# zju3dv/RelightableAvatar

Hardware: AMD Instinct MI355X
Metric: rays_per_sec (higher is better)
Workload: dtype f16

## Files before the change

### relightableavatar_amd/csrc/ra_api.cpp

```cpp
#include "ra_api_impl.hpp"
#include <cmath>

int check_ready(ra_ctx* c, const char* who) {
    if (!c) { ra_set_error(std::string(who) + ": null ctx"); return 1; }
    if (!c->have_weights) { ra_set_error(std::string(who) + ": weights not finalized"); return 1; }
    if (!c->have_frame) { ra_set_error(std::string(who) + ": no frame set (ra_set_frame)"); return 1; }
    if (hipSetDevice(c->device) != hipSuccess) { ra_set_error(std::string(who) + ": hipSetDevice failed"); return 1; }
    return 0;
}

static void zero_chunk_counters(ra_ctx* c, hipStream_t s) {
    hipMemsetAsync(icnt(c, 0), 0, CNT_ALL * sizeof(int), s);
    c->fc_next = 0;
    c->fc_wrapped = false;
    c->cnt_zero = true;
}
int* next_fine_counter(ra_ctx* c, hipStream_t s) {
    if (c->fc_next >= CNT_FC_SLOTS) {
        hipMemsetAsync(icnt(c, CNT_FC0), 0, CNT_FC_SLOTS * sizeof(int), s);
        c->fc_next = 0;
        c->fc_wrapped = true;
    }
    return icnt(c, CNT_FC0 + c->fc_next++);
}
// ... 90 lines not shown
static int key_mask_from(ra_ctx* c, const float* probe, int ph, int pw, hipStream_t s) {
    if (c->key_external) return 0;
    c->key_valid = false;
    if (!key_tier(c) || !probe) return 0;
    if (c->key_mask.ensure((size_t)c->n_lights) || c->key_share.ensure((size_t)c->n_lights * sizeof(float))) return 1;
    launch_key_lights(probe, 1, ph, pw, c->light_dir.as<float>(), c->light_area.as<float>(), c->n_lights, c->cfg.key_light_share, KEY_LIGHTS_MAX, 0,
                      c->key_share.as<float>(), c->key_mask.as<unsigned char>(), s);
    c->key_valid = true;
    return 0;
}

static void fine_level(ra_ctx* c, const MlpIO& io, int n, bool comp, hipStream_t s, int hint = -1) {
    const int nv = variant_size(n, hint);
    if (comp) {
        Timer t(c, s, T_K3C);
        launch_mlp_sdf_comp(c->host.geo, c->sarena_c.p, c->barena.as<float>(), c->fr, io, nv, s, c->k3cc_ok, grid_size(n, nv));
    } else {
        Timer t(c, s, k3_waves(nv) == 8 ? T_K3_WIDE : T_K3_NARROW);
        k3_launch(c, io, nv, s, grid_size(n, nv));
    }
}

static int hdq_pass(ra_ctx* c, const RaySet& rs, int n, float th, int smooth, float* sdf, hipStream_t s, int what = Q_OTHER,
                    const unsigned char* key = nullptr, int n_key = 0) {
    if (n <= 0) return 0;
    int err = 0;
    int* fine_idx = c->buf<int>("fine_idx", n, &err);
    float* bpts = c->buf<float>("fine_bpts", (size_t)n * 3, &err);
    if (err) return 1;
    HdqOut out{};
    out.sdf = sdf; out.fine_count = next_fine_counter(c, s); out.fine_idx = fine_idx; out.bpts = bpts;
    const int hint = fine_hint(c, c->fc_next - 1);
    int hint2 = -1;
    if (key && n_key > 0) {
        out.key = key;
        out.fine_idx2 = c->buf<int>("fine_idx_k", n_key, &err);
        out.bpts2 = c->buf<float>("fine_bpts_k", (size_t)n_key * 3, &err);
        if (err) return 1;
        out.fine_count2 = next_fine_counter(c, s);
        hint2 = fine_hint(c, c->fc_next - 1);
    }
    out.counters = dcnt(c);
    launch_hdq_coarse(c->fr, rs, n, th, c->cfg.blend_radius, out, s, c->cfg.use_geodesic_filter != 0);
    MlpIO io{};
    io.bpts = bpts; io.idx = fine_idx; io.count = out.fine_count; io.sdf = sdf; io.dist_th = th; io.smooth = smooth;
    io.resd_limit = c->cfg.resd_limit; io.counters = dcnt(c);
    fine_level(c, io, n, precise(c, what), s, hint);
    if (out.key) {
        io.bpts = out.bpts2; io.idx = out.fine_idx2; io.count = out.fine_count2;
        fine_level(c, io, n_key, true, s, hint2);
    }
    return 0;
}

int full_query(ra_ctx* c, FullIO io, int n, hipStream_t s) {
    const bool gated = c->gate && n > 65536;
    if (gated && c->gate->armed) RA_HIP(hipStreamWaitEvent(s, c->gate->done, 0));
    struct Release {
        ra_ctx* c; hipStream_t s; bool on;
        ~Release() { if (on) { hipEventRecord(c->gate->done, s); c->gate->armed = true; } }
    } release{c, s, gated};
    Timer t(c, s, T_K4);
    const int batch = c->cfg.k4_batch_slots > 0 ? c->cfg.k4_batch_slots : (1 << 20);
    const int cap = n < batch ? n : batch;
    int err = 0;
    char* tape = c->buf<char>("k4_tape", mlp_full_rev_tape_bytes(cap), &err);
    if (err) {
        ra_set_error("full query: no device memory for the activation tape (" + std::to_string(mlp_full_rev_tape_bytes(cap) >> 20) +
                     " MB): lower cfg.k4_batch_slots / cfg.volume_chunk_rays");
        return 1;
// ... 9 lines not shown
}

static int forward_pass(ra_ctx* c, const float* x, const float* v, int n, const int* n_dev, float th, float* raw, hipStream_t s) {
    if (n <= 0) return 0;
    int err = 0;
    const int C = raw_channels(c);
    int* fine_idx = c->buf<int>("fine_idx", n, &err);
    float* bpts = c->buf<float>("fine_bpts", (size_t)n * 3, &err);
    float* mats = c->buf<float>("fine_mats", (size_t)n * 24, &err);
    float* sdf = c->buf<float>("fwd_sdf", n, &err);
    if (err) return 1;
    RaySet rs{};
    rs.mode = 0; rs.x = x; rs.n_dev = n_dev;
    HdqOut out{};
    out.sdf = sdf; out.fine_count = next_fine_counter(c, s); out.fine_idx = fine_idx; out.bpts = bpts; out.mats = mats;
    out.raw_zero = raw; out.raw_C = C;
    out.counters = dcnt(c);
    launch_hdq_coarse(c->fr, rs, n, th, c->cfg.blend_radius, out, s, c->cfg.use_geodesic_filter != 0);
    FullIO io = full_io(c);
    io.bpts = bpts; io.mats = mats; io.view = v; io.idx = fine_idx; io.count = out.fine_count; io.raw = raw;
    return full_query(c, io, n, s);
}

static TraceState alloc_trace(ra_ctx* c, const std::string& p, int n, bool soft, int* err) {
    TraceState ts{};
    ts.t = c->buf<float>(p + "t", n, err);
    ts.d0 = c->buf<float>(p + "d0", n, err);
    ts.occ = c->buf<float>(p + "occ", n, err);
    ts.ot = c->buf<float>(p + "ot", n, err);
    ts.stuck = c->buf<unsigned char>(p + "stuck", n, err);
    if (!soft) {
        ts.dt = c->buf<float>(p + "dt", n, err);
        ts.st = c->buf<float>(p + "st", n, err);
        ts.cd = c->buf<float>(p + "cd", n, err);
        ts.off = c->buf<float>(p + "off", n, err);
        ts.rlx = c->buf<float>(p + "rlx", n, err);
    }
    return ts;
}

int sdf_points_precise(ra_ctx* c, int mode, const float* pts, int n, float dist_th, float* sdf, hipStream_t s) {
    if (n <= 0) return 0;
    if (mode == 2) {
        RaySet rs{};
        rs.mode = 0; rs.x = pts;
        return hdq_pass(c, rs, n, dist_th, 0, sdf, s, Q_PRECISE);
    }
    int err = 0;
    int* idx = c->buf<int>("fine_idx", n, &err);
    if (err) return 1;
    int* cnt = next_fine_counter(c, s);
    launch_iota(idx, n, cnt, s);
// ... 131 lines not shown
    ShadowGen g{};
    g.surf = st.surf; g.norm = st.norm_slots; g.acc = st.acc; g.hit_idx = st.hit_idx; g.hit_count = st.hit_count; g.ldir = c->light_dir.as<float>();
    for (int k = 0; k < 6; ++k) g.bbox[k] = st.bbox[k];
    g.n_boxes = st.n_boxes > 1 ? st.n_boxes : 0;
    for (int j = 0; j < g.n_boxes; ++j) {
        for (int k = 0; k < 6; ++k) g.boxes[j][k] = st.boxes[6 * j + k];
        g.box_start[j] = st.box_start[j];
    }
    if (g.n_boxes) g.box_start[g.n_boxes] = st.box_start[g.n_boxes];
    g.perm = g.n_boxes ? st.perm : nullptr;
    g.near_offset = st.near_offset; g.L = L; g.no_visibility = st.no_visibility; g.local_visibility = st.local_visibility;
    g.split_wide_groups = st.split_wide_groups ? 1 : 0;
    g.lvis = st.lvis; g.ldot = st.ldot;
    g.ray_count = icnt(c, CNT_RAYS);
    const bool traced = !(st.no_visibility || st.local_visibility);
    TraceState sh{};
    float* ssdf = nullptr;
    if (traced) {
        g.ray_pix = c->buf<int>("lv_pix", NR, &err);
        g.ray_light = c->buf<int>("lv_light", NR, &err);
        g.ray_slot = c->buf<int>("lv_slot", NR, &err);
        g.near_ = c->buf<float>("lv_near", NR, &err);
        g.far_ = c->buf<float>("lv_far", NR, &err);
        sh = alloc_trace(c, "sh_", (int)NR, shadow.soft_shadow != 0, &err);
        ssdf = c->buf<float>("sh_sdf", NR, &err);
    }
    const bool keyed = traced && key_tier(c) && c->key_valid;
    const size_t NK = keyed ? (size_t)P * (size_t)(L < KEY_LIGHTS_MAX ? L : KEY_LIGHTS_MAX) : 0;
    if (err) return 1;
    if (c->gate && c->gate->armed) RA_HIP(hipStreamWaitEvent(s, c->gate->done, 0));
    launch_shadow_gen(g, P, s, c->cnt_zero);
    c->cnt_zero = false;
    if (traced) {
        sh.near_ = g.near_; sh.far_ = g.far_; sh.tan_i = c->light_sharp.as<float>(); sh.light = g.ray_light;
        launch_trace_init(sh, (int)NR, g.ray_count, shadow, s);
        RaySet r2{};
        r2.mode = 2; r2.o = st.surf; r2.t = sh.t; r2.pix = g.ray_pix; r2.light = g.ray_light; r2.ldir = c->light_dir.as<float>();
        r2.n_dev = g.ray_count;
        r2.skip = c->cfg.query_skip ? sh.stuck : nullptr;
        r2.nn_hint = c->buf<int>("lv_nn", NR * 3, &err);
        if (err) return 1;
        for (int it = 0; it < shadow.iters; ++it) {
            r2.hint_valid = it > 0;
            r2.hint_src = it == 0 ? st.pix_nn : nullptr;
            r2.hint_src_index = it == 0 ? g.ray_pix : nullptr;
            if (hdq_pass(c, r2, (int)NR, shadow.dist_th, 1, ssdf, s, Q_OTHER, keyed ? c->key_mask.as<unsigned char>() : nullptr, (int)NK)) return 1;
            launch_trace_update(sh, ssdf, (int)NR, g.ray_count, it, shadow, s);
        }
        launch_shadow_scatter(sh.occ, g.ray_slot, g.ray_count, (int)NR, st.lvis, s);
        launch_accumulate(g.ray_count, &dcnt(c)->n_shadow_rays, s);
    }
    if (c->gate) { RA_HIP(hipEventRecord(c->gate->done, s)); c->gate->armed = true; }
    return 0;
}

int ra_begin_render(ra_ctx* c) {
    RA_CHECK(c, "ra_begin_render: null ctx");
    c->call_no = 0;
    return 0;
}

int ra_set_key_probes(ra_ctx* c, const float* probes, int n, int ph, int pw, int accumulate, void* stream) {
    RA_CHECK(c && n >= 0 && (n == 0 || (probes && ph > 0 && pw > 0)), "ra_set_key_probes: bad arguments");
    if (n == 0) { c->key_external = false; c->key_valid = false; return 0; }
    RA_CHECK(c->have_weights && c->n_lights > 0, "ra_set_key_probes: needs the relight network's light set (ra_finalize_weights)");
    RA_HIP(hipSetDevice(c->device));
    const bool acc = accumulate && c->key_external && c->key_valid;
    c->key_external = true;
    if (!key_tier(c)) { c->key_valid = false; return 0; }
    if (c->key_mask.ensure((size_t)c->n_lights) || c->key_share.ensure((size_t)c->n_lights * sizeof(float))) return 1;
    launch_key_lights(probes, n, ph, pw, c->light_dir.as<float>(), c->light_area.as<float>(), c->n_lights, c->cfg.key_light_share, KEY_LIGHTS_MAX,
                      acc ? 1 : 0, c->key_share.as<float>(), c->key_mask.as<unsigned char>(), (hipStream_t)stream);
    c->key_valid = true;
    RA_HIP(hipGetLastError());
    return 0;
// ... 289 lines not shown
```

### relightableavatar_amd/csrc/ra_hdq.hip

```cpp
#include "ra_kernels.hpp"
#include <type_traits>
#include <cstdlib>

namespace {

constexpr int KNN_THREADS = 256;

#ifdef RA_COARSE_TS
__device__ long long ra_coarse_ts[64 * 64 * 16 * 8];
extern "C" int ra_coarse_read_timestamps(long long* out) { return (int)hipMemcpyFromSymbol(out, HIP_SYMBOL(ra_coarse_ts), sizeof(ra_coarse_ts)); }
#define RA_CSTAMP(k) do { if (tsp) { __builtin_amdgcn_sched_barrier(0); if ((threadIdx.x & 63) == 0) tsp[k] = __builtin_readcyclecounter(); __builtin_amdgcn_sched_barrier(0); } } while (0)
#else
#define RA_CSTAMP(k) do { } while (0)
#endif
constexpr int VT = 2048;

__device__ __forceinline__ void inv3d(const float R[9], float M[9]) {
    M[0] = R[4] * R[8] - R[7] * R[5];
    M[3] = -R[3] * R[8] + R[6] * R[5];
    M[6] = R[3] * R[7] - R[6] * R[4];
    M[1] = -R[1] * R[8] + R[7] * R[2];
    M[4] = R[0] * R[8] - R[6] * R[2];
    M[7] = -R[0] * R[7] + R[6] * R[1];
    M[2] = R[1] * R[5] - R[4] * R[2];
// ... 186 lines not shown
    const float dy = fmaxf(fmaxf(ly - p[1], p[1] - hy), 0.f);
    const float dz = fmaxf(fmaxf(lz - p[2], p[2] - hz), 0.f);
    return dx * dx + dy * dy + dz * dz;
}

__device__ __forceinline__ float dist2(float dx, float dy, float dz) { return __fmaf_rn(dz, dz, __fmaf_rn(dx, dx, dy * dy)); }

__device__ __forceinline__ void knn_insert(float d, int id, float& d0, float& d1, float& d2, int& i0, int& i1, int& i2, bool dedup = false) {
    if (__builtin_expect(__ballot(d <= d2) == 0ull, 1)) return;
    bool fresh = true;
    if (dedup) fresh = (id != i0) & (id != i1) & (id != i2);
    const bool c2 = fresh && (d < d2 || (d == d2 && id < i2));
    const bool c1 = fresh && (d < d1 || (d == d1 && id < i1));
    const bool c0 = fresh && (d < d0 || (d == d0 && id < i0));
    const float nd2 = c1 ? d1 : (c2 ? d : d2);
    const int ni2 = c1 ? i1 : (c2 ? id : i2);
    const float nd1 = c0 ? d0 : (c1 ? d : d1);
    const int ni1 = c0 ? i0 : (c1 ? id : i1);
    d0 = c0 ? d : d0;
    i0 = c0 ? id : i0;
    d1 = nd1; i1 = ni1; d2 = nd2; i2 = ni2;
}

__device__ __forceinline__ void ray_point(const RaySet& rs, int i, float x[3]) {
    if (rs.mode == 0) {
        x[0] = rs.x[3 * i]; x[1] = rs.x[3 * i + 1]; x[2] = rs.x[3 * i + 2];
    } else if (rs.mode == 1) {
        const float t = rs.t[i];
        x[0] = rs.o[3 * i] + t * rs.d[3 * i];
        x[1] = rs.o[3 * i + 1] + t * rs.d[3 * i + 1];
        x[2] = rs.o[3 * i + 2] + t * rs.d[3 * i + 2];
    } else {
        const float t = rs.t[i];
        const int p = rs.pix[i], l = rs.light[i];
        x[0] = rs.o[3 * p] + t * rs.ldir[3 * l];
        x[1] = rs.o[3 * p + 1] + t * rs.ldir[3 * l + 1];
        x[2] = rs.o[3 * p + 2] + t * rs.ldir[3 * l + 2];
    }
}

template <bool BVH, int SPLIT, bool HINT = false>
__global__ __launch_bounds__(SPLIT == 1 ? KNN_THREADS : 64 * SPLIT) void hdq_coarse_kernel(FrameState fr, RaySet rs, int n_launch, float th, float inv2r2,
                                                                  HdqOut out, int dbg) {
    static_assert(SPLIT == 1 || (BVH && SPLIT >= 2 && SPLIT <= 16), "SPLIT > 1: the workgroup is SPLIT waves on the same 64 queries");
    constexpr int NT = SPLIT == 1 ? KNN_THREADS : 64 * SPLIT;
    __shared__ __attribute__((aligned(16))) unsigned char smem[BVH ? 16 : VT * 16];
#ifdef RA_COARSE_TS
    long long* tsp = blockIdx.x < 64 ? ra_coarse_ts + ((((dbg >> 8) & 63) * 64 + blockIdx.x) * 16 + (threadIdx.x >> 6)) * 8 : nullptr;
    dbg &= 255;
    if (tsp && (threadIdx.x & 63) == 0) { tsp[1] = tsp[2] = tsp[3] = tsp[4] = tsp[5] = tsp[6] = tsp[7] = 0; }
    RA_CSTAMP(0);
#endif
    const int n = rs.n_dev ? min(*rs.n_dev, n_launch) : n_launch;
    const int base = blockIdx.x * (SPLIT == 1 ? KNN_THREADS : 64);
    if (base >= n) return;
    if (blockIdx.x == 0 && threadIdx.x == 0 && out.counters) atomicAdd(&out.counters->n_coarse, (unsigned long long)n);
    const int i = base + (SPLIT == 1 ? threadIdx.x : (threadIdx.x & 63));
    const bool live_q = i < n && !(rs.skip && rs.skip[i < n ? i : 0]);
    bool live = live_q;
    if (__syncthreads_count(live_q) == 0) return;
    float x[3] = {0.f, 0.f, 0.f};
    if (live) ray_point(rs, i, x);
    const float xt[3] = {x[0] - fr.Th[0], x[1] - fr.Th[1], x[2] - fr.Th[2]};
    float p[3];
#pragma unroll
    for (int c = 0; c < 3; ++c) p[c] = xt[0] * fr.R[c] + xt[1] * fr.R[3 + c] + xt[2] * fr.R[6 + c];

    RA_CSTAMP(1);
    float d0 = 3.0e38f, d1 = 3.0e38f, d2 = 3.0e38f;
    int i0 = 0, i1 = 0, i2 = 0;
    if (dbg & 1) { d0 = 1e-4f; d1 = 2e-4f; d2 = 3e-4f; i0 = 0; i1 = 1; i2 = 2; }
    else if (BVH) {
        const int nl = fr.bvh_leaves, ns = fr.bvh_supers;
        if (!live) { d0 = d1 = d2 = -1.f; }
        const unsigned long long lm = __ballot(live);
        const int first = lm ? __ffsll((long long)lm) - 1 : 0;
        const int lane = threadIdx.x & 63;
        typedef float f2 __attribute__((ext_vector_type(2)));
        const f2 px2 = {p[0], p[0]}, py2 = {p[1], p[1]}, pz2 = {p[2], p[2]};
        constexpr bool hinted = HINT;
#ifdef RA_COARSE_TS
        int n_rare = 0;
#endif
        typedef float f8 __attribute__((ext_vector_type(8)));
        typedef float f4 __attribute__((ext_vector_type(4)));
// ... 279 lines not shown
void launch_bvh_build(const float4* pverts4, int n_verts, int* order, float* leaves, float4* sbox, int n_leaves, int n_supers, hipStream_t s) {
    hipLaunchKernelGGL(bvh_rank_kernel, dim3((n_verts + 63) / 64), dim3(BVH_THREADS), 0, s, pverts4, n_verts, order);
    hipLaunchKernelGGL(bvh_boxes_kernel, dim3(1), dim3(BVH_THREADS), 0, s, pverts4, order, n_verts, leaves, sbox, n_leaves, n_supers);
}

void launch_hdq_coarse(const FrameState& fr, const RaySet& rs, int n, float th, float blend_radius, const HdqOut& out,
                       hipStream_t s, bool geodesic) {
    if (n <= 0) return;
    const float inv2r2 = 1.f / (2.f * blend_radius * blend_radius);
    const dim3 grid((n + KNN_THREADS - 1) / KNN_THREADS);
    int dbg = 0, probe = 0, split_max = 196608;
#ifdef RA_TESTING
    static const int e_dbg = getenv("RA_COARSE_DBG") ? atoi(getenv("RA_COARSE_DBG")) : 0;
    static const int e_probe = getenv("RA_COARSE_PROBE") ? atoi(getenv("RA_COARSE_PROBE")) : 0;
    static const int e_split = getenv("RA_COARSE_SPLIT_MAX") ? atoi(getenv("RA_COARSE_SPLIT_MAX")) : 196608;
    dbg = e_dbg; probe = e_probe; split_max = e_split;
#endif
    if (!geodesic) dbg |= 32;
#ifdef RA_COARSE_TS
    static int launch_no = 0;
    dbg |= (launch_no++ & 63) << 8;
#endif
    const bool hint = (rs.nn_hint != nullptr && rs.hint_valid != 0) || rs.hint_src != nullptr;
    for (int pass = probe ? 0 : 1; pass < 2; ++pass) {
        const int d = pass == 0 ? probe : dbg;
        if (fr.bvh_leaves > 0 && n <= split_max)
        {
            const int groups = (n + 63) / 64;
            if (hint) {
                if (n <= split_max / 8) hipLaunchKernelGGL((hdq_coarse_kernel<true, 16, true>), dim3(groups), dim3(1024), 0, s, fr, rs, n, th, inv2r2, out, d);
                else if (n <= split_max / 2) hipLaunchKernelGGL((hdq_coarse_kernel<true, 8, true>), dim3(groups), dim3(512), 0, s, fr, rs, n, th, inv2r2, out, d);
                else hipLaunchKernelGGL((hdq_coarse_kernel<true, 4, true>), dim3(groups), dim3(256), 0, s, fr, rs, n, th, inv2r2, out, d);
            } else {
                if (n <= split_max / 8) hipLaunchKernelGGL((hdq_coarse_kernel<true, 16>), dim3(groups), dim3(1024), 0, s, fr, rs, n, th, inv2r2, out, d);
                else if (n <= split_max / 2) hipLaunchKernelGGL((hdq_coarse_kernel<true, 8>), dim3(groups), dim3(512), 0, s, fr, rs, n, th, inv2r2, out, d);
                else hipLaunchKernelGGL((hdq_coarse_kernel<true, 4>), dim3(groups), dim3(256), 0, s, fr, rs, n, th, inv2r2, out, d);
            }
        }
        else if (fr.bvh_leaves > 0 && hint) hipLaunchKernelGGL((hdq_coarse_kernel<true, 1, true>), grid, dim3(KNN_THREADS), 0, s, fr, rs, n, th, inv2r2, out, d);
        else if (fr.bvh_leaves > 0) hipLaunchKernelGGL((hdq_coarse_kernel<true, 1>), grid, dim3(KNN_THREADS), 0, s, fr, rs, n, th, inv2r2, out, d);
        else hipLaunchKernelGGL((hdq_coarse_kernel<false, 1>), grid, dim3(KNN_THREADS), 0, s, fr, rs, n, th, inv2r2, out, d);
        if (pass == 0) hipMemsetAsync(out.fine_count, 0, sizeof(int), s);
    }
}
```

### relightableavatar_amd/csrc/ra_kernels.hpp

```cpp
#pragma once
#include "ra_common.hpp"
#include "ra_lpips_pack.hpp"

struct RaySet {
    int mode;
    const float* x;
    const float* o;
    const float* d;
    const float* t;
    const int* pix;
    const int* light;
    const float* ldir;
    const int* n_dev;
    const unsigned char* skip;
    int* nn_hint;
    int hint_valid;
    const int* hint_src;
    const int* hint_src_index;
};

struct HdqOut {
    float* sdf;
    int* fine_count;
    int* fine_idx;
    float* bpts;
    float* mats;
    const unsigned char* key;
    int* fine_count2;
    int* fine_idx2;
    float* bpts2;
    float* raw_zero;
    int raw_C;
    float* dbg_sdf_batch;
    int* dbg_nn_batch;
    float* dbg_d2;
    float* dbg_tpts;
    float* dbg_bpts;
    float* dbg_mats;
    DevCounters* counters;
};

void launch_vert_blend(const float* weights, const float* A, const float* big_A, int n_verts, int n_bones, float* vertA,
                       hipStream_t s);
void launch_pack_verts(const float* pverts, int n_verts, float4* out, hipStream_t s);
void launch_fold_bias(const float* W, int ld, int col0, int ncond, const float* cond, const float* bias, float* out,
                      hipStream_t s);
void launch_bvh_build(const float4* pverts4, int n_verts, int* order, float* leaves, float4* sbox, int n_leaves, int n_supers, hipStream_t s);
int bvh_leaf_count(int n_verts);
int bvh_super_count(int n_leaves);
void launch_hdq_coarse(const FrameState& fr, const RaySet& rs, int n, float th, float blend_radius, const HdqOut& out,
                       hipStream_t s, bool geodesic = true);

struct TraceState {
    float *t, *d0, *dt, *st, *ot, *cd, *occ, *off, *rlx;
    const float *near_, *far_;
    const float* tan_i;
    const int* light;
    unsigned char* stuck;
};
void launch_trace_init(const TraceState& ts, int n, const int* n_dev, const ra_trace_params& p, hipStream_t s);

void launch_trace_update(const TraceState& ts, const float* sdf, int n, const int* n_dev, int iter,
                         const ra_trace_params& p, hipStream_t s);

void launch_surface_finish(const float* ray_o, const float* ray_d, const float* st, const float* occ, int P, float* surf,
                           float* depth, float* acc, int* hit_idx, int* hit_count, hipStream_t s, int* slot_of_ray = nullptr,
                           bool counter_is_zero = false);
void launch_slot_index(const int* hit_idx, const int* hit_count, int P, int* slot_of_ray, hipStream_t s);
struct MapJob { const float* src; float* dst; int C; int premul; int src_full; };
constexpr int RA_MAX_MAP_JOBS = 16;
struct EmitMaps { MapJob job[RA_MAX_MAP_JOBS]; long long end[RA_MAX_MAP_JOBS]; int n_jobs; const int* slot_of_ray; const float* acc; const int* perm; int P; };
void launch_emit_maps(const EmitMaps& m, hipStream_t s);
void launch_surface_samples(const float* surf, const float* ray_d, const int* hit_idx, const int* hit_count, int P, int S,
                            float range, float* x, float* v, int* n_out, hipStream_t s);
struct SurfaceMaps {
    float *cpts, *bpts, *resd, *norm, *albedo, *rough, *rgb;
    float* valbedo;
};
void launch_surface_composite(const float* raw, int C, int S, const int* hit_count, int P, int relight, const ra_config& cfg,
                              const SurfaceMaps& m, hipStream_t s);

constexpr int RA_MAX_BOXES = 32;
struct ShadowGen {
    const float* surf;
    const float* norm;
    const float* acc;
    const int* hit_idx;
    const int* hit_count;
    const float* ldir;
    float bbox[6];
    int n_boxes;
    float boxes[RA_MAX_BOXES][6];
    int box_start[RA_MAX_BOXES + 1];
    const int* perm;
    float near_offset;
    int L;
    int no_visibility, local_visibility;
    int split_wide_groups;
    float* lvis;
    float* ldot;
    int* ray_pix;
    int* ray_light;
    int* ray_slot;
    float *near_, *far_;
    int* ray_count;
};
void launch_key_lights(const float* probes, int n, int ph, int pw, const float* ldir, const float* area, int L, float share, int kmax,
                       int accumulate, float* smax, unsigned char* key, hipStream_t s);
void launch_gather_shard_rays(const long long* idx, int n, const float* ro, const float* rd, const float* nr, const float* fr, float* so, float* sd,
                              float* sn, float* sf, hipStream_t s);
void launch_scatter_rows(const float* src, const long long* src_idx, const long long* dst_idx, long long n, int C, float* dst, hipStream_t s);
void launch_shadow_gen(const ShadowGen& g, int P, hipStream_t s, bool counter_is_zero = false);
void launch_debug_aabb(const float* o, const float* d, int n, const float* bbox6, float* nr, float* fr, hipStream_t s);
void launch_debug_brdf(const float* p2l, const float* p2c, const float* nrm, const float* alb, const float* rough, int L, int N, const ra_config& cfg,
                       float* out, hipStream_t s);
size_t sort_hits_temp_bytes(int P);
int launch_sort_hits(const float* surf, const float* acc, int P, const float* bbox_min, unsigned* keys_in, unsigned* keys_out,
                     int* vals_in, int* hit_idx_out, void* temp, size_t temp_bytes, hipStream_t s);
void launch_shadow_scatter(const float* occ, const int* ray_slot, const int* ray_count, int max_rays, float* lvis, hipStream_t s);

struct ShadeIn {
    const float* ray_o;
    const float* surf;
    const int* idx;
    const int* count;
    int n;
    const float *norm, *albedo, *rough;
    const float *lvis, *ldot;
    const float *light_xyz, *light_area;
    int L;
    const float* probes;
    int n_probes, ph, pw;
    int want_spec;
    float *rgb, *shade, *spec;
};
void launch_shade(const ShadeIn& in, const ra_config& cfg, hipStream_t s);

constexpr int SHADE_BWD_MAX_GRID = 768;
constexpr size_t SHADE_BWD_LDS_BYTES = 65536;
struct ShadeBwd {
    const float *ray_o, *surf, *norm, *albedo, *rough;
    const float* lvis;
// ... 184 lines not shown
```

### relightableavatar_amd/csrc/ra_trace.hip

```cpp
#include "ra_kernels.hpp"
#include "ra_shade_dev.hpp"
#include <hipcub/hipcub.hpp>

namespace {

constexpr int TPB = 256;

__device__ __forceinline__ int live_count(const int* n_dev, int n) { return n_dev ? min(*n_dev, n) : n; }

__device__ __forceinline__ float linspace01(int s, int S) {
    if (S == 1) return 0.f;
    const float step = 1.f / (float)(S - 1);
    return (s < S / 2) ? (float)s * step : 1.f - (float)(S - 1 - s) * step;
}

__global__ void trace_init_kernel(TraceState ts, int n_launch, const int* n_dev, float offset, float relax) {
    const int i = blockIdx.x * TPB + threadIdx.x;
    if (i >= live_count(n_dev, n_launch)) return;
    const float nr = ts.near_[i], fr = ts.far_[i];
    ts.t[i] = nr;
    ts.d0[i] = 1e9f;
    ts.occ[i] = 1.f;
    if (ts.stuck) ts.stuck[i] = 0;
    if (ts.dt) ts.dt[i] = 1e9f;
    if (ts.st) ts.st[i] = fr;
    if (ts.ot) ts.ot[i] = fr;
    if (ts.cd) ts.cd[i] = 1e9f;
    if (ts.off) ts.off[i] = offset;
    if (ts.rlx) ts.rlx[i] = relax;
}

template <bool SOFT>
__global__ void trace_update_kernel(TraceState ts, const float* __restrict__ sdf, int n_launch, const int* n_dev, int iter,
                                    ra_trace_params p) {
    const int i = blockIdx.x * TPB + threadIdx.x;
    if (i >= live_count(n_dev, n_launch)) return;
    const float d1 = sdf[i];
    const float d0 = ts.d0[i];
    float t = ts.t[i];
    const float t_prev = t;
    float occ = ts.occ[i];
    const float nr = ts.near_[i], fr = ts.far_[i];
    float tan_i = p.tan_i;
    if (SOFT) {
        const float ti = ts.tan_i ? (ts.light ? ts.tan_i[ts.light[i]] : ts.tan_i[i]) : p.tan_i;
        tan_i = p.tan_i_multiplier * ti;
    }
    const float tan2 = (1.f / tan_i) * 2.f;
    float off = ts.off ? ts.off[i] : p.offset;
    float rlx = ts.rlx ? ts.rlx[i] : p.relax;
    float ot = ts.ot ? ts.ot[i] : 0.f;
    if (SOFT && p.clay_book && iter >= p.shadow_skip_iter) {
        const float dx0 = d0 + rlx * d0 + off;
        const float dx1 = d1 + rlx * d1 + off;
        const float dy = (dx1 * dx1) / (2.f * dx0);
        const float dx = (sqrtf(dx1 * dx1 - dy * dy) - off) / (1.f + rlx);
        const float den = fmaxf(fmaxf(t - dy, nr), p.eps);
        const float cls = fmaxf(dx, 0.f) / den / tan2;
        const bool msk = (cls < occ) && (dy < t) && (dx1 > 0.f) && (dx0 > 0.f) && (dx > 0.f) && (dy > 0.f) && (dy < dx0);
        if (msk) { ot = t - dy; occ = cls; }
    }
    if (iter >= p.shadow_skip_iter) {
        const float cls = fmaxf(d1, 0.f) / fmaxf(fmaxf(t, nr), p.eps) / tan2;
        if (cls < occ) { ot = t; occ = cls; }
    }
    if (!SOFT) {
        const float d1u = fabsf(d1), d0u = fabsf(d0);
        float st = ts.st[i], cd = ts.cd[i];
        const float dt = ts.dt[i];
        const float s0 = (d0 > 0.f) ? 1.f : ((d0 < 0.f) ? -1.f : 0.f);
        const float s1 = (d1 > 0.f) ? 1.f : ((d1 < 0.f) ? -1.f : 0.f);
        if (s0 != s1) {
            st = t - dt * fminf(fmaxf(d1u / (d0u + d1u + p.eps), 0.f), 1.f);
            off = 0.f;
            rlx = 0.f;
        }
        if (d1u < cd) { cd = d1u; st = t; }
        ts.st[i] = st;
        ts.cd[i] = cd;
        ts.off[i] = off;
        ts.rlx[i] = rlx;
    }
    const float dtn = d1 + rlx * d1 + off;
    t = t + dtn;
    t = fminf(t, fr);
    t = fmaxf(t, nr);
    if (ts.dt) ts.dt[i] = dtn;
    ts.t[i] = t;
    if (ts.stuck) ts.stuck[i] = (t == t_prev || (SOFT && occ == 0.f)) ? 1 : 0;
    ts.d0[i] = d1;
    ts.occ[i] = occ;
    if (ts.ot) ts.ot[i] = ot;
}

__global__ void surface_finish_kernel(const float* __restrict__ ro, const float* __restrict__ rd, const float* __restrict__ st,
                                      const float* __restrict__ occ, int P, float* __restrict__ surf, float* __restrict__ depth,
                                      float* __restrict__ acc, int* __restrict__ hit_idx, int* __restrict__ hit_count, int* __restrict__ slot_of_ray) {
    const int i = blockIdx.x * TPB + threadIdx.x;
    bool hit = false;
    if (i < P) {
        if (slot_of_ray) slot_of_ray[i] = -1;
        const float s = st[i];
        const float sx = ro[3 * i] + s * rd[3 * i], sy = ro[3 * i + 1] + s * rd[3 * i + 1], sz = ro[3 * i + 2] + s * rd[3 * i + 2];
        surf[3 * i] = sx; surf[3 * i + 1] = sy; surf[3 * i + 2] = sz;
        depth[i] = (sx - ro[3 * i]) / rd[3 * i];
        const float a = 1.f - occ[i];
        acc[i] = a;
        hit = a > 0.f;
    }
    const unsigned long long m = __ballot(hit);
    if (m == 0ull) return;
    const int lane = threadIdx.x & 63;
    int base = 0;
    if (lane == 0) base = atomicAdd(hit_count, __popcll(m));
    base = __shfl(base, 0);
// ... 271 lines not shown
                const int c0 = cnt[0][k], c1 = cnt[1][k];
                cnt[0][k] = tot; cnt[1][k] = tot + c0; tot += c0 + c1;
            }
        }
        cnt[0][NL] = tot ? atomicAdd(g.ray_count, tot) : 0;
    }
    __syncthreads();
    const int gbase = cnt[0][NL];
#pragma unroll
    for (int round = 0; round < ROUNDS; ++round) {
        const int ll = round * (TPB / 64) + wv;
        const bool trace = (tmask >> round) & 1u;
        const unsigned long long m = __ballot(trace);
        if (trace) {
            const int hf = lane >> 5;
            const unsigned mh = hf ? (unsigned)(m >> 32) : (unsigned)m;
            const int s = gbase + cnt[hf][ll] + __popc(mh & ((1u << (lane & 31)) - 1u));
            const int l = lc * SG_LIGHTS + ll;
            g.ray_pix[s] = r;
            g.ray_light[s] = l;
            g.ray_slot[s] = h * g.L + l;
            g.near_[s] = nrv[round];
            g.far_[s] = frv[round];
        }
    }
    const int col = threadIdx.x & (SG_LIGHTS - 1), l = lc * SG_LIGHTS + col;
    for (int row = threadIdx.x / SG_LIGHTS; row < 64; row += TPB / SG_LIGHTS) {
        const int hh = grp * 64 + row;
        if (hh < nh && l < g.L) {
            g.ldot[(size_t)hh * g.L + l] = t_ldot[row][col];
            g.lvis[(size_t)hh * g.L + l] = t_lvis[row][col];
        }
    }
}

__global__ void shadow_scatter_kernel(const float* __restrict__ occ, const int* __restrict__ ray_slot, const int* __restrict__ ray_count,
                                      int max_rays, float* __restrict__ lvis) {
    const int i = blockIdx.x * TPB + threadIdx.x;
    if (i >= min(*ray_count, max_rays)) return;
    lvis[ray_slot[i]] = occ[i];
}

__global__ __launch_bounds__(TPB) void key_lights_kernel(const float* __restrict__ probes, int n, int ph, int pw, const float* __restrict__ ldir,
                                                         const float* __restrict__ area, int L, float share, int kmax, int accumulate,
                                                         float* __restrict__ smax, unsigned char* __restrict__ key) {
    extern __shared__ float kl_w[];
    __shared__ float red[TPB / 64];
    for (int q = 0; q < n; ++q) {
        const float* img = probes + (size_t)q * ph * pw * 3;
        float part = 0.f;
        for (int l = threadIdx.x; l < L; l += TPB) {
            const float d[3] = {ldir[3 * l], ldir[3 * l + 1], ldir[3 * l + 2]};
            float c[3];
            sample_probe(img, ph, pw, d, c);
            float w = (c[0] + c[1] + c[2]) * (1.f / 3.f) * area[l];
            w = w > 0.f ? w : 0.f;
            kl_w[l] = w;
            part += w;
        }
#pragma unroll
        for (int sh = 32; sh > 0; sh >>= 1) part += __shfl_xor(part, sh);
        if ((threadIdx.x & 63) == 0) red[threadIdx.x >> 6] = part;
        __syncthreads();
// ... 762 lines not shown
int launch_gen_rays(const RayCam& cam, unsigned char* mask, int* pix_idx, int* count_dev, void* temp, size_t temp_bytes,
                    float* ray_o, float* ray_d, float* near, float* far, hipStream_t s) {
    const int n = cam.H * cam.W;
    if (n <= 0) { hipMemsetAsync(count_dev, 0, sizeof(int), s); return 0; }
    hipLaunchKernelGGL(ray_mask_kernel, grid_for(n), dim3(TPB), 0, s, cam, mask);
    if (hipcub::DeviceSelect::Flagged(temp, temp_bytes, hipcub::CountingInputIterator<int>(0), mask, pix_idx, count_dev, n, s) != hipSuccess) return 1;
    hipLaunchKernelGGL(ray_emit_kernel, grid_for(n), dim3(TPB), 0, s, cam, pix_idx, count_dev, ray_o, ray_d, near, far);
    return 0;
}

size_t sort_hits_temp_bytes(int P) {
    size_t bytes = 0;
    hipcub::DeviceRadixSort::SortPairs(nullptr, bytes, (const unsigned*)nullptr, (unsigned*)nullptr, (const int*)nullptr, (int*)nullptr, P);
    return bytes;
}

int launch_sort_hits(const float* surf, const float* acc, int P, const float* bbox_min, unsigned* keys_in, unsigned* keys_out,
                     int* vals_in, int* hit_idx_out, void* temp, size_t temp_bytes, hipStream_t s) {
    if (P <= 0) return 0;
    hipLaunchKernelGGL(hit_keys_kernel, grid_for(P), dim3(TPB), 0, s, surf, acc, P, bbox_min[0], bbox_min[1], bbox_min[2], keys_in, vals_in);
    return hipcub::DeviceRadixSort::SortPairs(temp, temp_bytes, keys_in, keys_out, vals_in, hit_idx_out, P, 0, 32, s) == hipSuccess ? 0 : 1;
}

void launch_shadow_scatter(const float* occ, const int* ray_slot, const int* ray_count, int max_rays, float* lvis, hipStream_t s) {
    if (max_rays <= 0) return;
    hipLaunchKernelGGL(shadow_scatter_kernel, grid_for(max_rays), dim3(TPB), 0, s, occ, ray_slot, ray_count, max_rays, lvis);
}

void launch_shade(const ShadeIn& in, const ra_config& cfg, hipStream_t s) {
    if (in.n <= 0) return;
    hipLaunchKernelGGL(shade_kernel, grid_for((long long)in.n * 64), dim3(TPB), 0, s, in, cfg);
}

void launch_scatter_maps(const int* hit_idx, const int* hit_count, int P, int premultiply, const float* acc_full, const float* src,
                         int C, float* dst, int src_full, const int* perm, hipStream_t s) {
    if (P <= 0) return;
    hipLaunchKernelGGL(scatter_maps_kernel, grid_for((long long)P * C), dim3(TPB), 0, s, hit_idx, hit_count, premultiply, acc_full, src, C, dst, src_full, perm);
}

int launch_sort_rays(const float* ro, const float* rd, const float* nr, const float* fr, int P, const float* bbox_min, unsigned* keys_in,
                     unsigned* keys_out, int* vals_in, int* perm, void* temp, size_t temp_bytes, float* so, float* sd, float* sn, float* sf,
                     hipStream_t s, float near_min, float far_max) {
    if (P <= 0) return 0;
    float* origin_dev = nullptr;
    if (!bbox_min) {
        origin_dev = reinterpret_cast<float*>(keys_out);
        hipLaunchKernelGGL(entry_min_kernel, dim3(1), dim3(1024), 0, s, ro, rd, nr, P, origin_dev);
    }
    hipLaunchKernelGGL(ray_keys_kernel, grid_for(P), dim3(TPB), 0, s, ro, rd, nr, P, bbox_min ? bbox_min[0] : 0.f, bbox_min ? bbox_min[1] : 0.f,
// ... 102 lines not shown
```

Before: 9.164 million.

## Fold shadow trace init/update into shadow gen, coarse query and scatter kernels

Trace initialization is moved into the shadow generation kernel. For soft shadows, each iteration's trace update is folded into the next coarse HDQ kernel, and the last update is folded into the scatter kernel. The ray count accumulate also moves into scatter, and the unused 'ot' buffer is dropped for soft shadows. The gate event is now recorded right after the last main fine pass, so the next frame can overlap with the keyed fine pass. This removes several small kernel launches and a global-memory round trip of trace state per iteration, at the cost of more complex coarse kernels, extra __syncthreads, and register pressure.

After: 9.247 million, median of 6. About the same (+0.9%).

```diff
diff --git a/relightableavatar_amd/csrc/ra_api.cpp b/relightableavatar_amd/csrc/ra_api.cpp
--- a/relightableavatar_amd/csrc/ra_api.cpp
+++ b/relightableavatar_amd/csrc/ra_api.cpp
@@ -136,7 +136,7 @@
 }
 
 static int hdq_pass(ra_ctx* c, const RaySet& rs, int n, float th, int smooth, float* sdf, hipStream_t s, int what = Q_OTHER,
-                    const unsigned char* key = nullptr, int n_key = 0) {
+                    const unsigned char* key = nullptr, int n_key = 0, bool release_gate = false) {
     if (n <= 0) return 0;
     int err = 0;
     int* fine_idx = c->buf<int>("fine_idx", n, &err);
@@ -160,6 +160,7 @@
     io.bpts = bpts; io.idx = fine_idx; io.count = out.fine_count; io.sdf = sdf; io.dist_th = th; io.smooth = smooth;
     io.resd_limit = c->cfg.resd_limit; io.counters = dcnt(c);
     fine_level(c, io, n, precise(c, what), s, hint);
+    if (release_gate && c->gate) { RA_HIP(hipEventRecord(c->gate->done, s)); c->gate->armed = true; }
     if (out.key) {
         io.bpts = out.bpts2; io.idx = out.fine_idx2; io.count = out.fine_count2;
         fine_level(c, io, n_key, true, s, hint2);
@@ -215,12 +216,12 @@
     return full_query(c, io, n, s);
 }
 
-static TraceState alloc_trace(ra_ctx* c, const std::string& p, int n, bool soft, int* err) {
+static TraceState alloc_trace(ra_ctx* c, const std::string& p, int n, bool soft, int* err, bool want_ot = true) {
     TraceState ts{};
     ts.t = c->buf<float>(p + "t", n, err);
     ts.d0 = c->buf<float>(p + "d0", n, err);
     ts.occ = c->buf<float>(p + "occ", n, err);
-    ts.ot = c->buf<float>(p + "ot", n, err);
+    if (!soft || want_ot) ts.ot = c->buf<float>(p + "ot", n, err);
     ts.stuck = c->buf<unsigned char>(p + "stuck", n, err);
     if (!soft) {
         ts.dt = c->buf<float>(p + "dt", n, err);
@@ -398,35 +399,44 @@
         g.ray_slot = c->buf<int>("lv_slot", NR, &err);
         g.near_ = c->buf<float>("lv_near", NR, &err);
         g.far_ = c->buf<float>("lv_far", NR, &err);
-        sh = alloc_trace(c, "sh_", (int)NR, shadow.soft_shadow != 0, &err);
+        sh = alloc_trace(c, "sh_", (int)NR, shadow.soft_shadow != 0, &err, false);
         ssdf = c->buf<float>("sh_sdf", NR, &err);
     }
     const bool keyed = traced && key_tier(c) && c->key_valid;
     const size_t NK = keyed ? (size_t)P * (size_t)(L < KEY_LIGHTS_MAX ? L : KEY_LIGHTS_MAX) : 0;
     if (err) return 1;
+    if (traced) {
+        sh.near_ = g.near_; sh.far_ = g.far_; sh.tan_i = c->light_sharp.as<float>(); sh.light = g.ray_light;
+        g.init = sh; g.init_offset = shadow.offset; g.init_relax = shadow.relax;
+    }
     if (c->gate && c->gate->armed) RA_HIP(hipStreamWaitEvent(s, c->gate->done, 0));
     launch_shadow_gen(g, P, s, c->cnt_zero);
     c->cnt_zero = false;
+    bool released = false;
     if (traced) {
-        sh.near_ = g.near_; sh.far_ = g.far_; sh.tan_i = c->light_sharp.as<float>(); sh.light = g.ray_light;
-        launch_trace_init(sh, (int)NR, g.ray_count, shadow, s);
         RaySet r2{};
         r2.mode = 2; r2.o = st.surf; r2.t = sh.t; r2.pix = g.ray_pix; r2.light = g.ray_light; r2.ldir = c->light_dir.as<float>();
         r2.n_dev = g.ray_count;
         r2.skip = c->cfg.query_skip ? sh.stuck : nullptr;
         r2.nn_hint = c->buf<int>("lv_nn", NR * 3, &err);
         if (err) return 1;
+        const bool fold = shadow.soft_shadow != 0;
+        PendingUpdate upd{};
+        upd.ts = sh; upd.sdf = ssdf; upd.p = shadow;
         for (int it = 0; it < shadow.iters; ++it) {
             r2.hint_valid = it > 0;
             r2.hint_src = it == 0 ? st.pix_nn : nullptr;
             r2.hint_src_index = it == 0 ? g.ray_pix : nullptr;
-            if (hdq_pass(c, r2, (int)NR, shadow.dist_th, 1, ssdf, s, Q_OTHER, keyed ? c->key_mask.as<unsigned char>() : nullptr, (int)NK)) return 1;
-            launch_trace_update(sh, ssdf, (int)NR, g.ray_count, it, shadow, s);
+            r2.upd = upd;
+            const bool last = it == shadow.iters - 1;
+            if (hdq_pass(c, r2, (int)NR, shadow.dist_th, 1, ssdf, s, Q_OTHER, keyed ? c->key_mask.as<unsigned char>() : nullptr, (int)NK, last)) return 1;
+            released = released || (last && NR > 0);
+            if (fold) { upd.on = 1; upd.iter = it; }
+            else launch_trace_update(sh, ssdf, (int)NR, g.ray_count, it, shadow, s);
         }
-        launch_shadow_scatter(sh.occ, g.ray_slot, g.ray_count, (int)NR, st.lvis, s);
-        launch_accumulate(g.ray_count, &dcnt(c)->n_shadow_rays, s);
-    }
-    if (c->gate) { RA_HIP(hipEventRecord(c->gate->done, s)); c->gate->armed = true; }
+        launch_shadow_scatter(upd, sh.occ, g.ray_slot, g.ray_count, (int)NR, st.lvis, &dcnt(c)->n_shadow_rays, s);
+    }
+    if (c->gate && !released) { RA_HIP(hipEventRecord(c->gate->done, s)); c->gate->armed = true; }
     return 0;
 }
 
diff --git a/relightableavatar_amd/csrc/ra_hdq.hip b/relightableavatar_amd/csrc/ra_hdq.hip
--- a/relightableavatar_amd/csrc/ra_hdq.hip
+++ b/relightableavatar_amd/csrc/ra_hdq.hip
@@ -1,4 +1,5 @@
 #include "ra_kernels.hpp"
+#include "ra_trace_dev.hpp"
 #include <type_traits>
 #include <cstdlib>
 
@@ -232,16 +233,16 @@
     d1 = nd1; i1 = ni1; d2 = nd2; i2 = ni2;
 }
 
-__device__ __forceinline__ void ray_point(const RaySet& rs, int i, float x[3]) {
+__device__ __forceinline__ void ray_point(const RaySet& rs, int i, float x[3], bool have_t = false, float t_new = 0.f) {
     if (rs.mode == 0) {
         x[0] = rs.x[3 * i]; x[1] = rs.x[3 * i + 1]; x[2] = rs.x[3 * i + 2];
     } else if (rs.mode == 1) {
-        const float t = rs.t[i];
+        const float t = have_t ? t_new : rs.t[i];
         x[0] = rs.o[3 * i] + t * rs.d[3 * i];
         x[1] = rs.o[3 * i + 1] + t * rs.d[3 * i + 1];
         x[2] = rs.o[3 * i + 2] + t * rs.d[3 * i + 2];
     } else {
-        const float t = rs.t[i];
+        const float t = have_t ? t_new : rs.t[i];
         const int p = rs.pix[i], l = rs.light[i];
         x[0] = rs.o[3 * p] + t * rs.ldir[3 * l];
         x[1] = rs.o[3 * p + 1] + t * rs.ldir[3 * l + 1];
@@ -266,11 +267,25 @@
     if (base >= n) return;
     if (blockIdx.x == 0 && threadIdx.x == 0 && out.counters) atomicAdd(&out.counters->n_coarse, (unsigned long long)n);
     const int i = base + (SPLIT == 1 ? threadIdx.x : (threadIdx.x & 63));
-    const bool live_q = i < n && !(rs.skip && rs.skip[i < n ? i : 0]);
+    const bool upd = HINT && rs.upd.on != 0;
+    float t_new = 0.f;
+    bool stuck_new = false;
+    if (upd) {
+        RayStep st;
+        if (i < n) st = trace_step<true>(rs.upd.ts, rs.upd.sdf, i, rs.upd.iter, rs.upd.p);
+        if (SPLIT > 1) __syncthreads();
+        if (i < n) {
+            if (SPLIT == 1 || threadIdx.x < 64) trace_step_store<true>(rs.upd.ts, i, st);
+            t_new = st.t;
+            stuck_new = st.stuck;
+        }
+    }
+    const bool skipped = i < n && rs.skip && ((upd && rs.skip == rs.upd.ts.stuck) ? stuck_new : rs.skip[i] != 0);
+    const bool live_q = i < n && !skipped;
     bool live = live_q;
     if (__syncthreads_count(live_q) == 0) return;
     float x[3] = {0.f, 0.f, 0.f};
-    if (live) ray_point(rs, i, x);
+    if (live) ray_point(rs, i, x, upd, t_new);
     const float xt[3] = {x[0] - fr.Th[0], x[1] - fr.Th[1], x[2] - fr.Th[2]};
     float p[3];
 #pragma unroll
@@ -596,24 +611,31 @@
     dbg |= (launch_no++ & 63) << 8;
 #endif
     const bool hint = (rs.nn_hint != nullptr && rs.hint_valid != 0) || rs.hint_src != nullptr;
+    RaySet rs_plain = rs;
+    rs_plain.upd.on = 0;
+    if (rs.upd.on && !(fr.bvh_leaves > 0 && hint)) launch_trace_update(rs.upd.ts, rs.upd.sdf, n, rs.n_dev, rs.upd.iter, rs.upd.p, s);
+    const bool fold = rs.upd.on && fr.bvh_leaves > 0 && hint;
+    bool folded = false;
     for (int pass = probe ? 0 : 1; pass < 2; ++pass) {
+        const RaySet& rq = (fold && !folded) ? rs : rs_plain;
+        folded = true;
         const int d = pass == 0 ? probe : dbg;
         if (fr.bvh_leaves > 0 && n <= split_max)
         {
             const int groups = (n + 63) / 64;
             if (hint) {
-                if (n <= split_max / 8) hipLaunchKernelGGL((hdq_coarse_kernel<true, 16, true>), dim3(groups), dim3(1024), 0, s, fr, rs, n, th, inv2r2, out, d);
-                else if (n <= split_max / 2) hipLaunchKernelGGL((hdq_coarse_kernel<true, 8, true>), dim3(groups), dim3(512), 0, s, fr, rs, n, th, inv2r2, out, d);
-                else hipLaunchKernelGGL((hdq_coarse_kernel<true, 4, true>), dim3(groups), dim3(256), 0, s, fr, rs, n, th, inv2r2, out, d);
+                if (n <= split_max / 8) hipLaunchKernelGGL((hdq_coarse_kernel<true, 16, true>), dim3(groups), dim3(1024), 0, s, fr, rq, n, th, inv2r2, out, d);
+                else if (n <= split_max / 2) hipLaunchKernelGGL((hdq_coarse_kernel<true, 8, true>), dim3(groups), dim3(512), 0, s, fr, rq, n, th, inv2r2, out, d);
+                else hipLaunchKernelGGL((hdq_coarse_kernel<true, 4, true>), dim3(groups), dim3(256), 0, s, fr, rq, n, th, inv2r2, out, d);
             } else {
-                if (n <= split_max / 8) hipLaunchKernelGGL((hdq_coarse_kernel<true, 16>), dim3(groups), dim3(1024), 0, s, fr, rs, n, th, inv2r2, out, d);
-                else if (n <= split_max / 2) hipLaunchKernelGGL((hdq_coarse_kernel<true, 8>), dim3(groups), dim3(512), 0, s, fr, rs, n, th, inv2r2, out, d);
-                else hipLaunchKernelGGL((hdq_coarse_kernel<true, 4>), dim3(groups), dim3(256), 0, s, fr, rs, n, th, inv2r2, out, d);
-            }
-        }
-        else if (fr.bvh_leaves > 0 && hint) hipLaunchKernelGGL((hdq_coarse_kernel<true, 1, true>), grid, dim3(KNN_THREADS), 0, s, fr, rs, n, th, inv2r2, out, d);
-        else if (fr.bvh_leaves > 0) hipLaunchKernelGGL((hdq_coarse_kernel<true, 1>), grid, dim3(KNN_THREADS), 0, s, fr, rs, n, th, inv2r2, out, d);
-        else hipLaunchKernelGGL((hdq_coarse_kernel<false, 1>), grid, dim3(KNN_THREADS), 0, s, fr, rs, n, th, inv2r2, out, d);
+                if (n <= split_max / 8) hipLaunchKernelGGL((hdq_coarse_kernel<true, 16>), dim3(groups), dim3(1024), 0, s, fr, rq, n, th, inv2r2, out, d);
+                else if (n <= split_max / 2) hipLaunchKernelGGL((hdq_coarse_kernel<true, 8>), dim3(groups), dim3(512), 0, s, fr, rq, n, th, inv2r2, out, d);
+                else hipLaunchKernelGGL((hdq_coarse_kernel<true, 4>), dim3(groups), dim3(256), 0, s, fr, rq, n, th, inv2r2, out, d);
+            }
+        }
+        else if (fr.bvh_leaves > 0 && hint) hipLaunchKernelGGL((hdq_coarse_kernel<true, 1, true>), grid, dim3(KNN_THREADS), 0, s, fr, rq, n, th, inv2r2, out, d);
+        else if (fr.bvh_leaves > 0) hipLaunchKernelGGL((hdq_coarse_kernel<true, 1>), grid, dim3(KNN_THREADS), 0, s, fr, rq, n, th, inv2r2, out, d);
+        else hipLaunchKernelGGL((hdq_coarse_kernel<false, 1>), grid, dim3(KNN_THREADS), 0, s, fr, rq, n, th, inv2r2, out, d);
         if (pass == 0) hipMemsetAsync(out.fine_count, 0, sizeof(int), s);
     }
 }
diff --git a/relightableavatar_amd/csrc/ra_kernels.hpp b/relightableavatar_amd/csrc/ra_kernels.hpp
--- a/relightableavatar_amd/csrc/ra_kernels.hpp
+++ b/relightableavatar_amd/csrc/ra_kernels.hpp
@@ -1,6 +1,22 @@
 #pragma once
 #include "ra_common.hpp"
 #include "ra_lpips_pack.hpp"
+
+struct TraceState {
+    float *t, *d0, *dt, *st, *ot, *cd, *occ, *off, *rlx;
+    const float *near_, *far_;
+    const float* tan_i;
+    const int* light;
+    unsigned char* stuck;
+};
+
+struct PendingUpdate {
+    int on;
+    int iter;
+    TraceState ts;
+    const float* sdf;
+    ra_trace_params p;
+};
 
 struct RaySet {
     int mode;
@@ -17,6 +33,7 @@
     int hint_valid;
     const int* hint_src;
     const int* hint_src_index;
+    PendingUpdate upd;
 };
 
 struct HdqOut {
@@ -51,13 +68,6 @@
 void launch_hdq_coarse(const FrameState& fr, const RaySet& rs, int n, float th, float blend_radius, const HdqOut& out,
                        hipStream_t s, bool geodesic = true);
 
-struct TraceState {
-    float *t, *d0, *dt, *st, *ot, *cd, *occ, *off, *rlx;
-    const float *near_, *far_;
-    const float* tan_i;
-    const int* light;
-    unsigned char* stuck;
-};
 void launch_trace_init(const TraceState& ts, int n, const int* n_dev, const ra_trace_params& p, hipStream_t s);
 
 void launch_trace_update(const TraceState& ts, const float* sdf, int n, const int* n_dev, int iter,
@@ -104,6 +114,8 @@
     int* ray_slot;
     float *near_, *far_;
     int* ray_count;
+    TraceState init;
+    float init_offset, init_relax;
 };
 void launch_key_lights(const float* probes, int n, int ph, int pw, const float* ldir, const float* area, int L, float share, int kmax,
                        int accumulate, float* smax, unsigned char* key, hipStream_t s);
@@ -117,7 +129,8 @@
 size_t sort_hits_temp_bytes(int P);
 int launch_sort_hits(const float* surf, const float* acc, int P, const float* bbox_min, unsigned* keys_in, unsigned* keys_out,
                      int* vals_in, int* hit_idx_out, void* temp, size_t temp_bytes, hipStream_t s);
-void launch_shadow_scatter(const float* occ, const int* ray_slot, const int* ray_count, int max_rays, float* lvis, hipStream_t s);
+void launch_shadow_scatter(const PendingUpdate& upd, const float* occ, const int* ray_slot, const int* ray_count, int max_rays, float* lvis,
+                           unsigned long long* total, hipStream_t s);
 
 struct ShadeIn {
     const float* ray_o;
diff --git a/relightableavatar_amd/csrc/ra_trace.hip b/relightableavatar_amd/csrc/ra_trace.hip
--- a/relightableavatar_amd/csrc/ra_trace.hip
+++ b/relightableavatar_amd/csrc/ra_trace.hip
@@ -1,5 +1,6 @@
 #include "ra_kernels.hpp"
 #include "ra_shade_dev.hpp"
+#include "ra_trace_dev.hpp"
 #include <hipcub/hipcub.hpp>
 
 namespace {
@@ -17,17 +18,7 @@
 __global__ void trace_init_kernel(TraceState ts, int n_launch, const int* n_dev, float offset, float relax) {
     const int i = blockIdx.x * TPB + threadIdx.x;
     if (i >= live_count(n_dev, n_launch)) return;
-    const float nr = ts.near_[i], fr = ts.far_[i];
-    ts.t[i] = nr;
-    ts.d0[i] = 1e9f;
-    ts.occ[i] = 1.f;
-    if (ts.stuck) ts.stuck[i] = 0;
-    if (ts.dt) ts.dt[i] = 1e9f;
-    if (ts.st) ts.st[i] = fr;
-    if (ts.ot) ts.ot[i] = fr;
-    if (ts.cd) ts.cd[i] = 1e9f;
-    if (ts.off) ts.off[i] = offset;
-    if (ts.rlx) ts.rlx[i] = relax;
+    trace_init_ray(ts, i, ts.near_[i], ts.far_[i], offset, relax);
 }
 
 template <bool SOFT>
@@ -35,62 +26,8 @@
                                     ra_trace_params p) {
     const int i = blockIdx.x * TPB + threadIdx.x;
     if (i >= live_count(n_dev, n_launch)) return;
-    const float d1 = sdf[i];
-    const float d0 = ts.d0[i];
-    float t = ts.t[i];
-    const float t_prev = t;
-    float occ = ts.occ[i];
-    const float nr = ts.near_[i], fr = ts.far_[i];
-    float tan_i = p.tan_i;
-    if (SOFT) {
-        const float ti = ts.tan_i ? (ts.light ? ts.tan_i[ts.light[i]] : ts.tan_i[i]) : p.tan_i;
-        tan_i = p.tan_i_multiplier * ti;
-    }
-    const float tan2 = (1.f / tan_i) * 2.f;
-    float off = ts.off ? ts.off[i] : p.offset;
-    float rlx = ts.rlx ? ts.rlx[i] : p.relax;
-    float ot = ts.ot ? ts.ot[i] : 0.f;
-    if (SOFT && p.clay_book && iter >= p.shadow_skip_iter) {
-        const float dx0 = d0 + rlx * d0 + off;
-        const float dx1 = d1 + rlx * d1 + off;
-        const float dy = (dx1 * dx1) / (2.f * dx0);
-        const float dx = (sqrtf(dx1 * dx1 - dy * dy) - off) / (1.f + rlx);
-        const float den = fmaxf(fmaxf(t - dy, nr), p.eps);
-        const float cls = fmaxf(dx, 0.f) / den / tan2;
-        const bool msk = (cls < occ) && (dy < t) && (dx1 > 0.f) && (dx0 > 0.f) && (dx > 0.f) && (dy > 0.f) && (dy < dx0);
-        if (msk) { ot = t - dy; occ = cls; }
-    }
-    if (iter >= p.shadow_skip_iter) {
-        const float cls = fmaxf(d1, 0.f) / fmaxf(fmaxf(t, nr), p.eps) / tan2;
-        if (cls < occ) { ot = t; occ = cls; }
-    }
-    if (!SOFT) {
-        const float d1u = fabsf(d1), d0u = fabsf(d0);
-        float st = ts.st[i], cd = ts.cd[i];
-        const float dt = ts.dt[i];
-        const float s0 = (d0 > 0.f) ? 1.f : ((d0 < 0.f) ? -1.f : 0.f);
-        const float s1 = (d1 > 0.f) ? 1.f : ((d1 < 0.f) ? -1.f : 0.f);
-        if (s0 != s1) {
-            st = t - dt * fminf(fmaxf(d1u / (d0u + d1u + p.eps), 0.f), 1.f);
-            off = 0.f;
-            rlx = 0.f;
-        }
-        if (d1u < cd) { cd = d1u; st = t; }
-        ts.st[i] = st;
-        ts.cd[i] = cd;
-        ts.off[i] = off;
-        ts.rlx[i] = rlx;
-    }
-    const float dtn = d1 + rlx * d1 + off;
-    t = t + dtn;
-    t = fminf(t, fr);
-    t = fmaxf(t, nr);
-    if (ts.dt) ts.dt[i] = dtn;
-    ts.t[i] = t;
-    if (ts.stuck) ts.stuck[i] = (t == t_prev || (SOFT && occ == 0.f)) ? 1 : 0;
-    ts.d0[i] = d1;
-    ts.occ[i] = occ;
-    if (ts.ot) ts.ot[i] = ot;
+    const RayStep r = trace_step<SOFT>(ts, sdf, i, iter, p);
+    trace_step_store<SOFT>(ts, i, r);
 }
 
 __global__ void surface_finish_kernel(const float* __restrict__ ro, const float* __restrict__ rd, const float* __restrict__ st,
@@ -408,6 +345,7 @@
             g.ray_slot[s] = h * g.L + l;
             g.near_[s] = nrv[round];
             g.far_[s] = frv[round];
+            if (g.init.t) trace_init_ray(g.init, s, nrv[round], frv[round], g.init_offset, g.init_relax);
         }
     }
     const int col = threadIdx.x & (SG_LIGHTS - 1), l = lc * SG_LIGHTS + col;
@@ -420,11 +358,13 @@
     }
 }
 
-__global__ void shadow_scatter_kernel(const float* __restrict__ occ, const int* __restrict__ ray_slot, const int* __restrict__ ray_count,
-                                      int max_rays, float* __restrict__ lvis) {
-    const int i = blockIdx.x * TPB + threadIdx.x;
+__global__ void shadow_scatter_kernel(PendingUpdate upd, const float* __restrict__ occ, const int* __restrict__ ray_slot,
+                                      const int* __restrict__ ray_count, int max_rays, float* __restrict__ lvis,
+                                      unsigned long long* __restrict__ total) {
+    const int i = blockIdx.x * TPB + threadIdx.x;
+    if (i == 0 && total) atomicAdd(total, (unsigned long long)*ray_count);
     if (i >= min(*ray_count, max_rays)) return;
-    lvis[ray_slot[i]] = occ[i];
+    lvis[ray_slot[i]] = upd.on ? trace_step<true>(upd.ts, upd.sdf, i, upd.iter, upd.p).occ : occ[i];
 }
 
 __global__ __launch_bounds__(TPB) void key_lights_kernel(const float* __restrict__ probes, int n, int ph, int pw, const float* __restrict__ ldir,
@@ -1233,9 +1173,10 @@
     return hipcub::DeviceRadixSort::SortPairs(temp, temp_bytes, keys_in, keys_out, vals_in, hit_idx_out, P, 0, 32, s) == hipSuccess ? 0 : 1;
 }
 
-void launch_shadow_scatter(const float* occ, const int* ray_slot, const int* ray_count, int max_rays, float* lvis, hipStream_t s) {
+void launch_shadow_scatter(const PendingUpdate& upd, const float* occ, const int* ray_slot, const int* ray_count, int max_rays, float* lvis,
+                           unsigned long long* total, hipStream_t s) {
     if (max_rays <= 0) return;
-    hipLaunchKernelGGL(shadow_scatter_kernel, grid_for(max_rays), dim3(TPB), 0, s, occ, ray_slot, ray_count, max_rays, lvis);
+    hipLaunchKernelGGL(shadow_scatter_kernel, grid_for(max_rays), dim3(TPB), 0, s, upd, occ, ray_slot, ray_count, max_rays, lvis, total);
 }
 
 void launch_shade(const ShadeIn& in, const ra_config& cfg, hipStream_t s) {
diff --git a/relightableavatar_amd/csrc/ra_trace_dev.hpp b/relightableavatar_amd/csrc/ra_trace_dev.hpp
--- /dev/null
+++ b/relightableavatar_amd/csrc/ra_trace_dev.hpp
@@ -0,0 +1,93 @@
+#pragma once
+#include "ra_kernels.hpp"
+
+struct RayStep {
+    float t, d0, occ, ot;
+    float dt, st, cd, off, rlx;
+    bool stuck;
+};
+
+__device__ __forceinline__ void trace_init_ray(const TraceState& ts, int i, float nr, float fr, float offset, float relax) {
+    ts.t[i] = nr;
+    ts.d0[i] = 1e9f;
+    ts.occ[i] = 1.f;
+    if (ts.stuck) ts.stuck[i] = 0;
+    if (ts.dt) ts.dt[i] = 1e9f;
+    if (ts.st) ts.st[i] = fr;
+    if (ts.ot) ts.ot[i] = fr;
+    if (ts.cd) ts.cd[i] = 1e9f;
+    if (ts.off) ts.off[i] = offset;
+    if (ts.rlx) ts.rlx[i] = relax;
+}
+
+template <bool SOFT>
+__device__ __forceinline__ RayStep trace_step(const TraceState& ts, const float* sdf, int i, int iter, const ra_trace_params& p) {
+    RayStep r;
+    const float d1 = sdf[i];
+    const float d0 = ts.d0[i];
+    float t = ts.t[i];
+    const float t_prev = t;
+    float occ = ts.occ[i];
+    const float nr = ts.near_[i], fr = ts.far_[i];
+    float tan_i = p.tan_i;
+    if (SOFT) {
+        const float ti = ts.tan_i ? (ts.light ? ts.tan_i[ts.light[i]] : ts.tan_i[i]) : p.tan_i;
+        tan_i = p.tan_i_multiplier * ti;
+    }
+    const float tan2 = (1.f / tan_i) * 2.f;
+    float off = ts.off ? ts.off[i] : p.offset;
+    float rlx = ts.rlx ? ts.rlx[i] : p.relax;
+    float ot = ts.ot ? ts.ot[i] : 0.f;
+    if (SOFT && p.clay_book && iter >= p.shadow_skip_iter) {
+        const float dx0 = d0 + rlx * d0 + off;
+        const float dx1 = d1 + rlx * d1 + off;
+        const float dy = (dx1 * dx1) / (2.f * dx0);
+        const float dx = (sqrtf(dx1 * dx1 - dy * dy) - off) / (1.f + rlx);
+        const float den = fmaxf(fmaxf(t - dy, nr), p.eps);
+        const float cls = fmaxf(dx, 0.f) / den / tan2;
+        const bool msk = (cls < occ) && (dy < t) && (dx1 > 0.f) && (dx0 > 0.f) && (dx > 0.f) && (dy > 0.f) && (dy < dx0);
+        if (msk) { ot = t - dy; occ = cls; }
+    }
+    if (iter >= p.shadow_skip_iter) {
+        const float cls = fmaxf(d1, 0.f) / fmaxf(fmaxf(t, nr), p.eps) / tan2;
+        if (cls < occ) { ot = t; occ = cls; }
+    }
+    r.st = 0.f; r.cd = 0.f;
+    if (!SOFT) {
+        const float d1u = fabsf(d1), d0u = fabsf(d0);
+        float st = ts.st[i], cd = ts.cd[i];
+        const float dt = ts.dt[i];
+        const float s0 = (d0 > 0.f) ? 1.f : ((d0 < 0.f) ? -1.f : 0.f);
+        const float s1 = (d1 > 0.f) ? 1.f : ((d1 < 0.f) ? -1.f : 0.f);
+        if (s0 != s1) {
+            st = t - dt * fminf(fmaxf(d1u / (d0u + d1u + p.eps), 0.f), 1.f);
+            off = 0.f;
+            rlx = 0.f;
+        }
+        if (d1u < cd) { cd = d1u; st = t; }
+        r.st = st; r.cd = cd;
+    }
+    const float dtn = d1 + rlx * d1 + off;
+    t = t + dtn;
+    t = fminf(t, fr);
+    t = fmaxf(t, nr);
+    r.stuck = t == t_prev || (SOFT && occ == 0.f);
+    r.t = t; r.d0 = d1; r.occ = occ; r.ot = ot; r.dt = dtn; r.off = off; r.rlx = rlx;
+    return r;
+}
+
+template <bool SOFT>
+__device__ __forceinline__ void trace_step_store(const TraceState& ts, int i, const RayStep& r) {
+    if (!SOFT) {
+        ts.st[i] = r.st;
+        ts.cd[i] = r.cd;
+        ts.off[i] = r.off;
+        ts.rlx[i] = r.rlx;
+    }
+    if (ts.dt) ts.dt[i] = r.dt;
+    ts.t[i] = r.t;
+    if (ts.stuck) ts.stuck[i] = r.stuck ? 1 : 0;
+    ts.d0[i] = r.d0;
+    ts.occ[i] = r.occ;
+    if (ts.ot) ts.ot[i] = r.ot;
+}
```
